# baryshnikova-lab/safepy

Hardware: AMD Instinct MI355X
Metric: node-attribute enrichments/sec (nodes x attrs x perms), compute_pvalues permutation test (higher is better)
Workload: dtype u1 (bit-sliced integer counts; f64 outputs)

## Files before the change

safepy_amd/csrc/check_hidden_regs.py:

```python
#!/usr/bin/env python3
import glob
import os
import re
import subprocess
import sys
import tempfile

LLVM = os.environ.get('SAFE_LLVM_BIN', '/opt/rocm/lib/llvm/bin')
KERNEL = '_Z19k_permtest_bits_blkILi8E'
RESERVED = range(112, 120)
OWN = re.compile(r'^(global_load_dwordx4 v\[(112:115|116:119)\], v\d+, s\[\d+:\d+\]'
                 r'|v_and_b32_e32 v\d+, 0xffff, v11[2-9]'
                 r'|v_lshrrev_b32_e32 v\d+, 16, v11[2-9])\s*$')


def names_reserved(text):
    for lo, hi in re.findall(r'\bv\[(\d+):(\d+)\]', text):
        if int(lo) <= RESERVED[-1] and int(hi) >= RESERVED[0]:
            return True
    for single in re.findall(r'\bv(\d+)\b', text):
        if int(single) in RESERVED:
            return True
    return False


def hipcc_version():
    try:
        out = subprocess.run([os.environ.get('HIPCC', '/opt/rocm/bin/hipcc'), '--version'], capture_output=True, text=True).stdout
        hip = re.search(r'HIP version: (\S+)', out)
        clang = re.search(r'clang version (\S+)', out)
        return 'hipcc %s (clang %s)' % (hip.group(1) if hip else '?', clang.group(1) if clang else '?')
    except OSError:
        return 'hipcc ?'


def write_header(path, checked, note):
    with open(path, 'w') as f:
        f.write('// generated by check_hidden_regs.py at build time\n')
        f.write('#define SAFE_HIDDEN_REGS_CHECKED %d\n' % (1 if checked else 0))
        f.write('#define SAFE_BUILD_COMPILER "%s"\n' % hipcc_version().replace('"', "'"))
        f.write('#define SAFE_BUILD_NOTE "%s"\n' % note.replace('"', "'"))


def main():
    obj, header = sys.argv[1], sys.argv[2]
    objdump, readobj = os.path.join(LLVM, 'llvm-objdump'), os.path.join(LLVM, 'llvm-readobj')
    if not os.path.exists(objdump):
        write_header(header, False, 'hidden-register check NOT run (no llvm-objdump): the kernel form without hidden registers is used')
        print('check_hidden_regs: no llvm-objdump at %s -- the library will run the form without hidden registers' % objdump)
        return 0
    with tempfile.TemporaryDirectory() as tmp:
        local = os.path.join(tmp, 'enrich.o')
        with open(obj, 'rb') as src, open(local, 'wb') as dst:
            dst.write(src.read())
        subprocess.run([objdump, '--offloading', local], capture_output=True, cwd=tmp, check=True)
        kernels, uses, foreign, vgprs = set(), 0, [], {}
        arch = os.environ.get('SAFE_ARCH', 'gfx950')
        for co in sorted(glob.glob(os.path.join(tmp, 'enrich.o.*%s*' % arch))):
            text = subprocess.run([objdump, '-d', '--no-show-raw-insn', co], capture_output=True, text=True, check=True).stdout
            if KERNEL not in text:
                continue
            sym = None
            for line in text.split('\n'):
                m = re.match(r'^[0-9a-f]+ <(.+)>:$', line)
                if m:
                    sym = m.group(1)
                    continue
                ins = line.split('//')[0].strip()
                if sym and sym.startswith(KERNEL) and names_reserved(ins):
                    kernels.add(sym)
                    uses += 1
                    if not OWN.match(ins):
                        foreign.append((sym[:60], ins))
            if os.path.exists(readobj):
                notes = subprocess.run([readobj, '--notes', co], capture_output=True, text=True).stdout
                for blk in notes.split('- .agpr_count')[1:]:
                    name = re.search(r'\.name:\s+(\S+)', blk)
                    count = re.search(r'\.vgpr_count:\s+(\d+)', blk)
                    if name and count and name.group(1).startswith(KERNEL):
                        vgprs[name.group(1)] = int(count.group(1))
    if not kernels or uses < 1000:
        print('check_hidden_regs: FAILED -- the stream kernels were not found in %s (%d uses of v112..v119)' % (obj, uses))
        return 1
    if foreign:
        print('check_hidden_regs: FAILED -- the compiler uses the reserved registers v112..v119 itself:')
        for sym, ins in foreign[:10]:
            print('   %s: %s' % (sym, ins))
        return 1
    stream = {k: v for k, v in vgprs.items() if k in kernels}
    bad = {k: v for k, v in stream.items() if v != 120}
    if bad:
        print('check_hidden_regs: FAILED -- kernel descriptors with a VGPR count other than 120: %s' % bad)
        return 1
    write_header(header, True, 'hidden-register check passed: %d kernels, %d uses of v112..v119, all the id stream\'s own; %d descriptors at 120 VGPRs'
                 % (len(kernels), uses, len(stream)))
    print('check_hidden_regs: ok (%d stream kernels, %d uses of v112..v119, %d descriptors checked)' % (len(kernels), uses, len(stream)))
    return 0


if __name__ == '__main__':
    sys.exit(main())
```

safepy_amd/csrc/enrich.hip:

```cpp
#include <algorithm>
#include <cmath>
#include <numeric>

#include "common.h"
#include "hyp_math.h"

template <typename T, int BN, int PLANES>
__global__ __launch_bounds__(256) void k_tile_prep(const void *__restrict__ raw, int64_t n, int64_t rs, int64_t cs,
                                                   int64_t col0, int64_t mloc, int64_t n_tiles,
                                                   double *__restrict__ bt) {
    const int64_t idx = static_cast<int64_t>(blockIdx.x) * 256 + threadIdx.x;
    const int64_t total = n_tiles * (n + 1) * BN;
    if (idx >= total) return;
    const int c = static_cast<int>(idx % BN);
    const int64_t row = (idx / BN) % (n + 1);
    const int64_t tile = idx / (static_cast<int64_t>(BN) * (n + 1));
    const int64_t j = tile * BN + c;
    double v = 0.0, v2 = 0.0, nn = 0.0;
    if (row < n && j < mloc) {
        const T x = reinterpret_cast<const T *>(raw)[row * rs + (col0 + j) * cs];
        if (x == x) {
            v = static_cast<double>(x);
            v2 = static_cast<double>(static_cast<T>(x * x));
            nn = 1.0;
// ... 365 lines not shown
}

#define BT_LV 10
static_assert(BT_LV == BITS_PLAN_LV, "the planning header (bits_plan.h) cuts the forms at the same number of levels");

typedef uint4 __attribute__((may_alias)) uint4_alias;

__device__ __forceinline__ uint32_t xor3(uint32_t a, uint32_t b, uint32_t c) { return __builtin_amdgcn_bitop3_b32(a, b, c, 0x96); }
__device__ __forceinline__ uint32_t maj3(uint32_t a, uint32_t b, uint32_t c) { return __builtin_amdgcn_bitop3_b32(a, b, c, 0xE8); }

template <int LV>
__device__ __forceinline__ uint32_t vadd8(uint32_t (&s)[LV], const uint32_t (&x)[8]) {
    uint32_t t2a = maj3(s[0], x[0], x[1]);
    s[0] = xor3(s[0], x[0], x[1]);
    uint32_t t2b = maj3(s[0], x[2], x[3]);
    s[0] = xor3(s[0], x[2], x[3]);
    const uint32_t t4a = maj3(s[1], t2a, t2b);
    s[1] = xor3(s[1], t2a, t2b);
    t2a = maj3(s[0], x[4], x[5]);
    s[0] = xor3(s[0], x[4], x[5]);
    t2b = maj3(s[0], x[6], x[7]);
    s[0] = xor3(s[0], x[6], x[7]);
    const uint32_t t4b = maj3(s[1], t2a, t2b);
    s[1] = xor3(s[1], t2a, t2b);
    const uint32_t t8 = maj3(s[2], t4a, t4b);
    s[2] = xor3(s[2], t4a, t4b);
    return t8;
}

template <int LV>
__device__ __forceinline__ void vripple(uint32_t (&s)[LV], uint32_t t8) {
#pragma unroll
    for (int l = 3; l < LV; ++l) {
        const uint32_t c = s[l] & t8;
        s[l] ^= t8;
        t8 = c;
    }
}

typedef const __attribute__((address_space(3))) unsigned short *lds_u16_ptr;
typedef unsigned int u32x2 __attribute__((ext_vector_type(2)));
typedef const __attribute__((address_space(3))) u32x2 *lds_u2_ptr;

template <int CL>
__device__ __forceinline__ void vcount(uint32_t (&c)[CL], uint32_t &pend, uint32_t m) {
#pragma unroll
    for (int l = 0; l < 3; ++l) {
        uint32_t k;
        asm("v_and_b32 %0, %1, %2\n\tv_xor_b32 %1, %1, %2" : "=&v"(k), "+v"(c[l]) : "v"(m));
        m = k;
    }
    pend |= m;
}

template <int CL>
__device__ __forceinline__ void vflush(uint32_t (&c)[CL], uint32_t &pend) {
    uint32_t m = pend;
#pragma unroll
    for (int l = 3; l < CL; ++l) {
        uint32_t k;
        asm("v_and_b32 %0, %1, %2\n\tv_xor_b32 %1, %1, %2" : "=&v"(k), "+v"(c[l]) : "v"(m));
        m = k;
    }
    pend = 0;
}

template <int NT = 256>
__device__ __forceinline__ void load_word_column(uint2 *__restrict__ T, const uint2 *__restrict__ src, int64_t n) {
    constexpr int UNL = NT > 256 ? 4 : 16;
    for (int64_t r0 = threadIdx.x; r0 <= n; r0 += NT * UNL) {
        uint2 v[UNL];
#pragma unroll
        for (int u = 0; u < UNL; ++u) {
            const int64_t r = r0 + u * NT;
            v[u] = src[r <= n ? r : n];
        }
#pragma unroll
        for (int u = 0; u < UNL; ++u) {
            const int64_t r = r0 + u * NT;
            if (r <= n) T[r] = v[u];
        }
    }
}

template <int LEVELS>
__device__ __forceinline__ unsigned int vextract(const uint32_t (&c)[LEVELS], int bit) {
    unsigned int v = 0;
#pragma unroll
    for (int l = 0; l < LEVELS; ++l) v |= ((c[l] >> bit) & 1u) << l;
    return v;
}

__device__ __forceinline__ void transpose32(uint32_t (&a)[32]) {
#pragma unroll
    for (int j = 16; j != 0; j >>= 1) {
        const uint32_t m = j == 16 ? 0x0000FFFFu : j == 8 ? 0x00FF00FFu : j == 4 ? 0x0F0F0F0Fu : j == 2 ? 0x33333333u : 0x55555555u;
#pragma unroll
        for (int k = 0; k < 32; ++k) {
            if ((k & j) == 0) {
                const uint32_t t = ((a[k] >> j) ^ a[k + j]) & m;
                a[k] ^= t << j;
                a[k + j] ^= t;
            }
        }
    }
}

__global__ __launch_bounds__(256) void k_permute_cols(const uint16_t *__restrict__ cur16, int64_t stride16,
                                                      const uint16_t *__restrict__ sell_col2, int64_t entries,
                                                      int64_t entries_pad, int64_t p0, int64_t count, uint32_t pad_off,
                                                      uint16_t *__restrict__ out, int sh) {
    extern __shared__ uint16_t row[];
    const int64_t q = blockIdx.y;
    if (q >= count) return;
    const uint4 *src = reinterpret_cast<const uint4 *>(cur16 + (p0 + q) * stride16);
    for (int64_t v = threadIdx.x; v < stride16 / 8; v += 256) reinterpret_cast<uint4 *>(row)[v] = src[v];
    __syncthreads();
    const int64_t e0 = static_cast<int64_t>(blockIdx.x) * 4096;
#pragma unroll
    for (int j = 0; j < 2; ++j) {
        const int64_t e = e0 + (j * 256 + threadIdx.x) * 8;
        if (e >= entries_pad) break;
        uint4 o;
        if (e + 8 <= entries) {
            const uint4 c = *reinterpret_cast<const uint4 *>(sell_col2 + e);
            const uint32_t a0 = row[(c.x & 0xFFFFu) >> 1], a1 = row[c.x >> 17], a2 = row[(c.y & 0xFFFFu) >> 1], a3 = row[c.y >> 17];
            const uint32_t a4 = row[(c.z & 0xFFFFu) >> 1], a5 = row[c.z >> 17], a6 = row[(c.w & 0xFFFFu) >> 1], a7 = row[c.w >> 17];
            o.x = (a0 << sh) | (a1 << (16 + sh));
            o.y = (a2 << sh) | (a3 << (16 + sh));
            o.z = (a4 << sh) | (a5 << (16 + sh));
            o.w = (a6 << sh) | (a7 << (16 + sh));
        } else {
            uint32_t v[8];
#pragma unroll
            for (int u = 0; u < 8; ++u) v[u] = e + u < entries ? static_cast<uint32_t>(row[sell_col2[e + u] >> 1]) << sh : pad_off;
            o.x = (v[0] & 0xFFFFu) | (v[1] << 16);
            o.y = (v[2] & 0xFFFFu) | (v[3] << 16);
            o.z = (v[4] & 0xFFFFu) | (v[5] << 16);
            o.w = (v[6] & 0xFFFFu) | (v[7] << 16);
        }
        *reinterpret_cast<uint4 *>(out + q * entries_pad + e) = o;
    }
}

template <int SHIFT, int LV>
__device__ __forceinline__ void bits_accumulate_ids(const uint16_t *__restrict__ ids, int wdt, uint32_t t_addr,
                                                    uint32_t (&s0)[LV], uint32_t (&s1)[LV]) {
#pragma unroll
    for (int l = 0; l < LV; ++l) s0[l] = s1[l] = 0;
    uint32_t c[8];
#pragma unroll
    for (int u = 0; u < 8; ++u) c[u] = ids[u * 64];
    const uint16_t *pc = ids + 8 * 64;
    for (int t0 = 0; t0 < wdt; t0 += 8, pc += 8 * 64) {
        uint32_t r[8];
#pragma unroll
        for (int u = 0; u < 8; ++u) r[u] = (c[u] << SHIFT) + t_addr;
#pragma unroll
        for (int u = 0; u < 8; ++u) c[u] = pc[u * 64];
        uint32_t x0[8], x1[8];
#pragma unroll
        for (int u = 0; u < 8; ++u) {
            const u32x2 w = *(lds_u2_ptr)(uintptr_t)(r[u]);
            x0[u] = w.x;
            x1[u] = w.y;
        }
// ... 246 lines not shown
}

template <int LV>
__device__ __forceinline__ void vripple_lv(uint32_t (&s)[LV], uint32_t t8) {
#pragma unroll
    for (int l = 3; l < LV; ++l) {
        uint32_t c;
        asm("v_and_b32 %0, %1, %2\n\tv_xor_b32 %1, %1, %2" : "=&v"(c), "+v"(s[l]) : "v"(t8));
        t8 = c;
    }
}

template <int LV>
__device__ __forceinline__ uint32_t vripple_low(uint32_t (&s)[LV], uint32_t t8) {
#pragma unroll
    for (int l = 3; l < 5 && l < LV; ++l) {
        uint32_t c;
        asm("v_and_b32 %0, %1, %2\n\tv_xor_b32 %1, %1, %2" : "=&v"(c), "+v"(s[l]) : "v"(t8));
        t8 = c;
    }
    return t8;
}
template <int LV>
__device__ __forceinline__ void vripple_high(uint32_t (&s)[LV], uint32_t t32) {
#pragma unroll
    for (int l = 5; l < LV; ++l) {
        uint32_t c;
        asm("v_and_b32 %0, %1, %2\n\tv_xor_b32 %1, %1, %2" : "=&v"(c), "+v"(s[l]) : "v"(t32));
        t32 = c;
    }
}

template <int LV, int SHIFT, int GATHER, bool RIP2 = false>
__device__ __forceinline__ void blk_add8(u32x4 &c, const u32x4 *__restrict__ refill, uint32_t (&s0)[LV], uint32_t (&s1)[LV]) {
    uint32_t a[8];
    a[0] = (c.x & 0xFFFFu) << SHIFT;
    a[1] = (c.x >> 16) << SHIFT;
    a[2] = (c.y & 0xFFFFu) << SHIFT;
    a[3] = (c.y >> 16) << SHIFT;
    a[4] = (c.z & 0xFFFFu) << SHIFT;
    a[5] = (c.z >> 16) << SHIFT;
    a[6] = (c.w & 0xFFFFu) << SHIFT;
    a[7] = (c.w >> 16) << SHIFT;
    c = *refill;
    if (GATHER == 2) {
        const uint32_t lane_bits = (__builtin_amdgcn_mbcnt_hi(~0u, __builtin_amdgcn_mbcnt_lo(~0u, 0u)) & 31u) << 3;
#pragma unroll
        for (int u = 0; u < 8; ++u) a[u] = (a[u] & 0xFF00u) | lane_bits;
    }
    uint32_t x0[8], x1[8];
#pragma unroll
    for (int u = 0; u < 8; ++u) {
        if (GATHER) {
            const u32x2 w = *(lds_u2_ptr)(uintptr_t)(a[u]);
            x0[u] = w.x;
            x1[u] = w.y;
        } else {
            x0[u] = a[u];
            x1[u] = a[u] >> 3;
        }
    }
    const uint32_t e0 = vadd8_lv<LV>(s0, x0);
    const uint32_t e1 = vadd8_lv<LV>(s1, x1);
    if (__builtin_amdgcn_ballot_w64((e0 | e1) != 0)) {
        if constexpr (RIP2 && LV >= 8) {
            const uint32_t c0 = vripple_low<LV>(s0, e0), c1 = vripple_low<LV>(s1, e1);
            if (__builtin_amdgcn_ballot_w64((c0 | c1) != 0)) {
                vripple_high<LV>(s0, c0);
                vripple_high<LV>(s1, c1);
            }
        } else {
            vripple_lv<LV>(s0, e0);
            vripple_lv<LV>(s1, e1);
        }
    }
}

#pragma clang diagnostic push
#pragma clang diagnostic ignored "-Winline-asm"
template <int Q>
__device__ __forceinline__ void stream_fetch(const u32x4 *base, uint32_t lane_off) {
    if (Q == 0) asm volatile("global_load_dwordx4 v[112:115], %0, %1" : : "v"(lane_off), "s"(base) : "v112", "v113", "v114", "v115");
    else asm volatile("global_load_dwordx4 v[116:119], %0, %1" : : "v"(lane_off), "s"(base) : "v116", "v117", "v118", "v119");
}

template <int LV, int GATHER, bool RIP2, int Q>
__device__ __forceinline__ void blk_add8s(const u32x4 *base, uint32_t lane_off, uint32_t (&s0)[LV], uint32_t (&s1)[LV]) {
    uint32_t a[8];
    if (Q == 0)
        asm volatile("s_waitcnt vmcnt(1)\n\tv_and_b32 %0, 0xffff, v112\n\tv_lshrrev_b32 %1, 16, v112\n\tv_and_b32 %2, 0xffff, v113\n\t"
                     "v_lshrrev_b32 %3, 16, v113\n\tv_and_b32 %4, 0xffff, v114\n\tv_lshrrev_b32 %5, 16, v114\n\t"
                     "v_and_b32 %6, 0xffff, v115\n\tv_lshrrev_b32 %7, 16, v115"
                     : "=v"(a[0]), "=v"(a[1]), "=v"(a[2]), "=v"(a[3]), "=v"(a[4]), "=v"(a[5]), "=v"(a[6]), "=v"(a[7]));
    else
        asm volatile("s_waitcnt vmcnt(1)\n\tv_and_b32 %0, 0xffff, v116\n\tv_lshrrev_b32 %1, 16, v116\n\tv_and_b32 %2, 0xffff, v117\n\t"
                     "v_lshrrev_b32 %3, 16, v117\n\tv_and_b32 %4, 0xffff, v118\n\tv_lshrrev_b32 %5, 16, v118\n\t"
                     "v_and_b32 %6, 0xffff, v119\n\tv_lshrrev_b32 %7, 16, v119"
                     : "=v"(a[0]), "=v"(a[1]), "=v"(a[2]), "=v"(a[3]), "=v"(a[4]), "=v"(a[5]), "=v"(a[6]), "=v"(a[7]));
    stream_fetch<Q>(base, lane_off);
    if (GATHER == 2) {
        const uint32_t lane_bits = (__builtin_amdgcn_mbcnt_hi(~0u, __builtin_amdgcn_mbcnt_lo(~0u, 0u)) & 31u) << 3;
#pragma unroll
        for (int u = 0; u < 8; ++u) a[u] = (a[u] & 0xFF00u) | lane_bits;
    }
    uint32_t x0[8], x1[8];
#pragma unroll
    for (int u = 0; u < 8; ++u) {
        if (GATHER) {
            const u32x2 w = *(lds_u2_ptr)(uintptr_t)(a[u]);
            x0[u] = w.x;
            x1[u] = w.y;
        } else {
            x0[u] = a[u];
            x1[u] = a[u] >> 3;
        }
    }
    const uint32_t e0 = vadd8_lv<LV>(s0, x0);
    const uint32_t e1 = vadd8_lv<LV>(s1, x1);
    if (__builtin_amdgcn_ballot_w64((e0 | e1) != 0)) {
        if constexpr (RIP2 && LV >= 8) {
            const uint32_t c0 = vripple_low<LV>(s0, e0), c1 = vripple_low<LV>(s1, e1);
            if (__builtin_amdgcn_ballot_w64((c0 | c1) != 0)) {
                vripple_high<LV>(s0, c0);
                vripple_high<LV>(s1, c1);
            }
        } else {
            vripple_lv<LV>(s0, e0);
            vripple_lv<LV>(s1, e1);
        }
    }
}

constexpr int HALF_MAX_LV = 8;
template <int Q>
__device__ __forceinline__ void stream_ids_lo(uint32_t (&a)[4]) {
    if (Q == 0)
        asm volatile("s_waitcnt vmcnt(1)\n\tv_and_b32 %0, 0xffff, v112\n\tv_lshrrev_b32 %1, 16, v112\n\tv_and_b32 %2, 0xffff, v113\n\t"
                     "v_lshrrev_b32 %3, 16, v113" : "=v"(a[0]), "=v"(a[1]), "=v"(a[2]), "=v"(a[3]));
    else
        asm volatile("s_waitcnt vmcnt(1)\n\tv_and_b32 %0, 0xffff, v116\n\tv_lshrrev_b32 %1, 16, v116\n\tv_and_b32 %2, 0xffff, v117\n\t"
                     "v_lshrrev_b32 %3, 16, v117" : "=v"(a[0]), "=v"(a[1]), "=v"(a[2]), "=v"(a[3]));
}
template <int Q>
__device__ __forceinline__ void stream_ids_hi(uint32_t (&a)[4]) {
    if (Q == 0)
        asm volatile("v_and_b32 %0, 0xffff, v114\n\tv_lshrrev_b32 %1, 16, v114\n\tv_and_b32 %2, 0xffff, v115\n\t"
                     "v_lshrrev_b32 %3, 16, v115" : "=v"(a[0]), "=v"(a[1]), "=v"(a[2]), "=v"(a[3]));
    else
        asm volatile("v_and_b32 %0, 0xffff, v118\n\tv_lshrrev_b32 %1, 16, v118\n\tv_and_b32 %2, 0xffff, v119\n\t"
                     "v_lshrrev_b32 %3, 16, v119" : "=v"(a[0]), "=v"(a[1]), "=v"(a[2]), "=v"(a[3]));
}
template <int GATHER>
__device__ __forceinline__ void gather4(uint32_t (&a)[4], uint32_t (&x0)[4], uint32_t (&x1)[4]) {
    if (GATHER == 2) {
        const uint32_t lane_bits = (__builtin_amdgcn_mbcnt_hi(~0u, __builtin_amdgcn_mbcnt_lo(~0u, 0u)) & 31u) << 3;
#pragma unroll
        for (int u = 0; u < 4; ++u) a[u] = (a[u] & 0xFF00u) | lane_bits;
    }
#pragma unroll
    for (int u = 0; u < 4; ++u) {
        if (GATHER) {
            const u32x2 w = *(lds_u2_ptr)(uintptr_t)(a[u]);
            x0[u] = w.x;
            x1[u] = w.y;
        } else {
            x0[u] = a[u];
            x1[u] = a[u] >> 3;
        }
    }
}
template <int LV>
__device__ __forceinline__ uint32_t vadd4_lv(uint32_t (&s)[LV], const uint32_t (&x)[4]) {
    const uint32_t t2a = maj3(s[0], x[0], x[1]);
    s[0] = xor3(s[0], x[0], x[1]);
    const uint32_t t2b = maj3(s[0], x[2], x[3]);
    s[0] = xor3(s[0], x[2], x[3]);
    const uint32_t t4 = maj3(s[1], t2a, t2b);
    s[1] = xor3(s[1], t2a, t2b);
    return t4;
}
template <int LV, int GATHER, bool RIP2, int Q>
__device__ __forceinline__ void blk_step(const u32x4 *base, uint32_t lane_off, uint32_t (&s0)[LV], uint32_t (&s1)[LV], uint32_t (&X0)[4],
                                         uint32_t (&X1)[4]) {
    uint32_t a[4], Y0[4], Y1[4];
    stream_ids_hi<Q>(a);
    stream_fetch<Q>(base, lane_off);
    gather4<GATHER>(a, Y0, Y1);
    const uint32_t f0 = vadd4_lv<LV>(s0, X0), f1 = vadd4_lv<LV>(s1, X1);
    stream_ids_lo<1 - Q>(a);
    gather4<GATHER>(a, X0, X1);
    const uint32_t h0 = vadd4_lv<LV>(s0, Y0), h1 = vadd4_lv<LV>(s1, Y1);
    const uint32_t e0 = maj3(s0[2], f0, h0), e1 = maj3(s1[2], f1, h1);
    s0[2] = xor3(s0[2], f0, h0);
    s1[2] = xor3(s1[2], f1, h1);
    if (__builtin_amdgcn_ballot_w64((e0 | e1) != 0)) {
        if constexpr (RIP2 && LV >= 8) {
            const uint32_t c0 = vripple_low<LV>(s0, e0), c1 = vripple_low<LV>(s1, e1);
            if (__builtin_amdgcn_ballot_w64((c0 | c1) != 0)) {
                vripple_high<LV>(s0, c0);
                vripple_high<LV>(s1, c1);
            }
        } else {
            vripple_lv<LV>(s0, e0);
            vripple_lv<LV>(s1, e1);
        }
    }
}

template <int LV, int SHIFT, int GATHER, bool RIP2 = false>
__device__ __forceinline__ void blk_sum(const u32x4 *__restrict__ ids, int lane, int nblk, uint32_t (&s0)[LV], uint32_t (&s1)[LV]) {
#pragma unroll
    for (int l = 0; l < LV; ++l) s0[l] = s1[l] = 0;
    u32x4 ca = ids[lane], cb = ids[64 + lane];
    const u32x4 *pc = ids + 128 + lane;
    int b = 0;
    constexpr int STEP = GATHER == 3 ? 0 : 128;
    for (; b + 1 < nblk; b += 2, pc += STEP) {
        blk_add8<LV, SHIFT, GATHER, RIP2>(ca, pc, s0, s1);
        blk_add8<LV, SHIFT, GATHER, RIP2>(cb, pc + 64, s0, s1);
    }
    if (b < nblk) blk_add8<LV, SHIFT, GATHER, RIP2>(ca, pc, s0, s1);
}

template <int LV, int CL, int DBG>
__device__ __forceinline__ void blk_task_core(const uint32_t *__restrict__ obs, const u32x4 *__restrict__ perm_ids, int64_t perm_stride,
                                              int lane, int nblk, int np, uint32_t (&g0)[CL], uint32_t (&g1)[CL], uint32_t (&l0)[CL],
                                              uint32_t (&l1)[CL]) {
    constexpr int GATHER = (DBG & 1) ? 0 : (DBG & 8) ? 2 : (DBG & 16) ? 3 : 1;
    uint32_t o0[LV], o1[LV];
#pragma unroll
    for (int l = 0; l < LV; ++l) {
        o0[l] = obs[l * 64 + lane];
        o1[l] = obs[(BT_LV + l) * 64 + lane];
    }
    uint32_t gp0 = 0, gp1 = 0, lp0 = 0, lp1 = 0;
    constexpr bool STREAM = (DBG & 256) == 0;
    u32x4 ca{}, cb{};
    const bool single = !STREAM && LV == 4 && nblk == 1 && GATHER != 3;
    if (single) {
        ca = perm_ids[lane];
        cb = perm_ids[(np > 1 ? perm_stride : 0) + lane];
    }
    const uint32_t pf_hi = static_cast<uint32_t>(__builtin_amdgcn_readfirstlane(static_cast<int>(reinterpret_cast<uint64_t>(perm_ids) >> 32)));
    const uint32_t pf_lo = static_cast<uint32_t>(__builtin_amdgcn_readfirstlane(static_cast<int>(reinterpret_cast<uint64_t>(perm_ids))));
    const u32x4 *pf_base = reinterpret_cast<const u32x4 *>((static_cast<uint64_t>(pf_hi) << 32) | static_cast<uint64_t>(pf_lo));
    uint32_t pf = 0;
    int pf_left = nblk, pf_perms = np;
    const uint32_t pf_stride = static_cast<uint32_t>(perm_stride) * 16u, pf_wrap = pf_stride - static_cast<uint32_t>(nblk) * 1024u;
    const uint32_t lane_off = static_cast<uint32_t>(lane) * 16u;
    auto pf_next = [&]() __attribute__((always_inline)) {
        if (GATHER == 3) return;
        pf += 1024u;
        if (__builtin_expect(--pf_left == 0, 0)) {
            asm volatile("");
            pf_left = nblk;
            pf += pf_wrap;
            if (--pf_perms == 0) {
                pf_perms = 1;
                pf -= pf_stride;
            }
        }
    };
    auto settle = [&](int p, uint32_t (&s0)[LV], uint32_t (&s1)[LV]) __attribute__((always_inline)) {
        if (DBG & 4) {
            g0[0] ^= s0[0] ^ s0[LV - 1];
            g1[0] ^= s1[0] ^ s1[LV - 1];
            return;
        }
        uint32_t gt0 = 0, gt1 = 0, lt0 = 0, lt1 = 0;
#pragma unroll
        for (int l = 0; l < LV; ++l) {
            lt0 = __builtin_amdgcn_bitop3_b32(s0[l], o0[l], lt0, 0x8E);
            gt0 = __builtin_amdgcn_bitop3_b32(s0[l], o0[l], gt0, 0xB2);
            lt1 = __builtin_amdgcn_bitop3_b32(s1[l], o1[l], lt1, 0x8E);
            gt1 = __builtin_amdgcn_bitop3_b32(s1[l], o1[l], gt1, 0xB2);
        }
        vcount<CL>(g0, gp0, gt0);
        vcount<CL>(g1, gp1, gt1);
        vcount<CL>(l0, lp0, lt0);
        vcount<CL>(l1, lp1, lt1);
        if ((p & 7) == 7) {
            vflush<CL>(g0, gp0);
            vflush<CL>(g1, gp1);
            vflush<CL>(l0, lp0);
            vflush<CL>(l1, lp1);
        }
    };
    if (STREAM) {
        constexpr bool R2 = (DBG & 32) == 0;
        constexpr bool HALF = (DBG & 512) == 0 && LV <= HALF_MAX_LV;
        stream_fetch<0>(pf_base, pf + lane_off);
        pf_next();
        stream_fetch<1>(pf_base, pf + lane_off);
        pf_next();
        uint32_t X0[4] = {0, 0, 0, 0}, X1[4] = {0, 0, 0, 0};
        if (HALF) {
            uint32_t a[4];
            stream_ids_lo<0>(a);
            gather4<GATHER>(a, X0, X1);
        }
        auto blockA = [&](uint32_t (&s0)[LV], uint32_t (&s1)[LV]) __attribute__((always_inline)) {
            if (HALF) blk_step<LV, GATHER, R2, 0>(pf_base, pf + lane_off, s0, s1, X0, X1);
            else blk_add8s<LV, GATHER, R2, 0>(pf_base, pf + lane_off, s0, s1);
            pf_next();
        };
        auto blockB = [&](uint32_t (&s0)[LV], uint32_t (&s1)[LV]) __attribute__((always_inline)) {
            if (HALF) blk_step<LV, GATHER, R2, 1>(pf_base, pf + lane_off, s0, s1, X0, X1);
            else blk_add8s<LV, GATHER, R2, 1>(pf_base, pf + lane_off, s0, s1);
            pf_next();
        };
        const int pairs = nblk >> 1;
        auto add_pairs = [&](uint32_t (&s0)[LV], uint32_t (&s1)[LV]) __attribute__((always_inline)) {
            for (int i = 0; i < pairs; ++i) {
                blockA(s0, s1);
                blockB(s0, s1);
            }
        };
        if (nblk & 1) {
            int p = 0;
            for (; p + 1 < np; p += 2) {
                uint32_t s0[LV], s1[LV];
#pragma unroll
                for (int l = 0; l < LV; ++l) s0[l] = s1[l] = 0;
                add_pairs(s0, s1);
                blockA(s0, s1);
                settle(p, s0, s1);
#pragma unroll
                for (int l = 0; l < LV; ++l) s0[l] = s1[l] = 0;
                blockB(s0, s1);
                add_pairs(s0, s1);
                settle(p + 1, s0, s1);
            }
            if (p < np) {
                uint32_t s0[LV], s1[LV];
#pragma unroll
                for (int l = 0; l < LV; ++l) s0[l] = s1[l] = 0;
                add_pairs(s0, s1);
                blockA(s0, s1);
                settle(p, s0, s1);
            }
        } else {
            for (int p = 0; p < np; ++p) {
                uint32_t s0[LV], s1[LV];
#pragma unroll
                for (int l = 0; l < LV; ++l) s0[l] = s1[l] = 0;
                add_pairs(s0, s1);
                settle(p, s0, s1);
            }
        }
    } else {
        for (int p = 0; p < np; ++p, perm_ids += perm_stride) {
            uint32_t s0[LV], s1[LV];
            if (single) {
#pragma unroll
                for (int l = 0; l < LV; ++l) s0[l] = s1[l] = 0;
                const u32x4 *ahead = perm_ids + (p + 2 < np ? 2 * perm_stride : 0) + lane;
                if (p & 1) blk_add8<LV, 0, GATHER>(cb, ahead, s0, s1);
                else blk_add8<LV, 0, GATHER>(ca, ahead, s0, s1);
            } else
                blk_sum<LV, 0, GATHER, (DBG & 32) == 0>(perm_ids, lane, nblk, s0, s1);
            settle(p, s0, s1);
        }
    }
    vflush<CL>(g0, gp0);
    vflush<CL>(g1, gp1);
    vflush<CL>(l0, lp0);
    vflush<CL>(l1, lp1);
    if (STREAM) asm volatile("s_waitcnt vmcnt(0)" : : : "v112", "v113", "v114", "v115", "v116", "v117", "v118", "v119");
}
#pragma clang diagnostic pop

template <int LV, int CL, int DBG>
__device__ __forceinline__ void blk_task(const uint32_t *__restrict__ obs, const u32x4 *__restrict__ perm_ids, int64_t perm_stride,
                                         int lane, int nblk, int np, uint32_t (&g0)[CL], uint32_t (&g1)[CL], uint32_t (&l0)[CL],
                                         uint32_t (&l1)[CL]) {
    blk_task_core<LV, CL, DBG>(obs, perm_ids, perm_stride, lane, nblk, np, g0, g1, l0, l1);
}

template <int LV>
__device__ __forceinline__ void observed_wave(const u32x4 *__restrict__ ids, int lane, int nblk, uint32_t *__restrict__ obs,
                                              uint32_t (&oo0)[BT_LV], uint32_t (&oo1)[BT_LV]) {
    uint32_t o0[LV], o1[LV];
    blk_sum<LV, 2, 1>(ids, lane, nblk, o0, o1);
#pragma unroll
    for (int l = 0; l < BT_LV; ++l) {
        oo0[l] = l < LV ? o0[l < LV ? l : 0] : 0u;
        oo1[l] = l < LV ? o1[l < LV ? l : 0] : 0u;
        obs[l * 64 + lane] = oo0[l];
        obs[(BT_LV + l) * 64 + lane] = oo1[l];
    }
}

__global__ __launch_bounds__(256) void k_bits_observed(int64_t n, const int32_t *__restrict__ sell_row,
                                                       const int64_t *__restrict__ slice_off,
                                                       const int32_t *__restrict__ slice_width,
                                                       const uint16_t *__restrict__ sell_col2b, int64_t n_slices,
                                                       const uint2 *__restrict__ bbits, int64_t mloc,
                                                       uint32_t *__restrict__ obs, double *__restrict__ ns_out) {
    extern __shared__ unsigned int lds[];
    uint2 *T = reinterpret_cast<uint2 *>(lds);
    if ((uint32_t)(uintptr_t)((__attribute__((address_space(3))) unsigned int *)lds) != 0u) __builtin_trap();
    const int wave = __builtin_amdgcn_readfirstlane(threadIdx.x >> 6), lane = threadIdx.x & 63;
    const int64_t wg = blockIdx.x, s = static_cast<int64_t>(blockIdx.y) * 4 + wave;
    load_word_column(T, bbits + wg * (n + 1), n);
    __syncthreads();
    if (s >= n_slices) return;
    const int wdt = __builtin_amdgcn_readfirstlane(slice_width[s]);
    const u32x4 *ids = reinterpret_cast<const u32x4 *>(sell_col2b) + slice_off[s] / 8;
    uint32_t *my_obs = obs + (wg * n_slices + s) * (2 * BT_LV * 64);
    uint32_t oo0[BT_LV], oo1[BT_LV];
    if (wdt <= 8) observed_wave<4>(ids, lane, wdt >> 3, my_obs, oo0, oo1);
    else if (wdt <= 56) observed_wave<6>(ids, lane, wdt >> 3, my_obs, oo0, oo1);
    else if (wdt <= 248) observed_wave<8>(ids, lane, wdt >> 3, my_obs, oo0, oo1);
    else if (wdt <= 504) observed_wave<9>(ids, lane, wdt >> 3, my_obs, oo0, oo1);
    else observed_wave<BT_LV>(ids, lane, wdt >> 3, my_obs, oo0, oo1);
    if (ns_out) {
        const int32_t row = sell_row[s * 64 + lane];
        uint16_t *tile = reinterpret_cast<uint16_t *>(lds + 2 * ((n + 2) & ~int64_t(1)) + 4) + wave * (64 * 66);
#pragma unroll
        for (int half = 0; half < 2; ++half)
#pragma unroll
            for (int bit = 0; bit < 32; ++bit)
                tile[lane * 66 + half * 32 + bit] = static_cast<uint16_t>(half ? vextract<BT_LV>(oo1, bit) : vextract<BT_LV>(oo0, bit));
        const int64_t jc = wg * 64 + lane;
#pragma unroll 8
        for (int r = 0; r < 64; ++r) {
            const int32_t row_r = __shfl(row, r);
            if (row_r >= 0 && jc < mloc) ns_out[static_cast<int64_t>(row_r) * mloc + jc] = static_cast<double>(tile[r * 66 + lane]);
        }
    }
}

template <int CL, bool PLAIN_STORE = false>
__device__ __forceinline__ void flush_counters(const uint32_t (&g0)[CL], const uint32_t (&g1)[CL], const uint32_t (&l0)[CL],
                                               const uint32_t (&l1)[CL], unsigned int *__restrict__ gl_counts, int64_t col0,
                                               int64_t mloc, int64_t n_pad, int64_t spos, bool active) {
#pragma unroll
    for (int half = 0; half < 2; ++half) {
        uint32_t m[32];
#pragma unroll
        for (int l = 0; l < 16; ++l) {
            m[l] = l < CL ? (half ? g1[l < CL ? l : 0] : g0[l < CL ? l : 0]) : 0u;
            m[16 + l] = l < CL ? (half ? l1[l < CL ? l : 0] : l0[l < CL ? l : 0]) : 0u;
        }
        transpose32(m);
        const int64_t c_first = col0 + half * 32;
        const int n_valid = static_cast<int>(mloc - c_first < 32 ? (mloc - c_first > 0 ? mloc - c_first : 0) : 32);
        int64_t off = c_first * n_pad + spos;
#pragma unroll
        for (int bit = 0; bit < 32; ++bit) {
            asm volatile("" : "+v"(off));
            if (PLAIN_STORE) {
                if (bit < n_valid && active && m[bit]) gl_counts[off] = m[bit];
            } else if (bit < n_valid && active && m[bit]) atomicAdd(gl_counts + off, m[bit]);
            off += n_pad;
        }
    }
}

constexpr int BLK_TRACE_MAX = 1 << 17;
__device__ unsigned long long g_blk_trace[BLK_TRACE_MAX * 8];
__device__ unsigned int g_blk_trace_n;

template <int CL, int DBG>
__device__ __forceinline__ void bits_blk_body(

    int64_t n, const uint16_t *__restrict__ ids_p, int64_t entries_pad, const int32_t *__restrict__ sell_row,
    const int64_t *__restrict__ slice_off, const int32_t *__restrict__ slice_width,
    const uint32_t *__restrict__ obs, int64_t n_slices, const uint2 *__restrict__ bbits, BitsQueues qs,
    const int4 *__restrict__ tasks, int64_t p_base, int64_t p_limit, unsigned int *__restrict__ queue, int64_t mloc,
    unsigned int *__restrict__ gl_counts, int64_t n_pad) {
    extern __shared__ unsigned int lds[];
    const int64_t t_words = 2 * ((n + 2) & ~int64_t(1));
    uint2 *T = reinterpret_cast<uint2 *>(lds);
    int *slot_box = reinterpret_cast<int *>(lds + t_words);
    if ((uint32_t)(uintptr_t)((__attribute__((address_space(3))) unsigned int *)lds) != 0u) __builtin_trap();
    const int wave = __builtin_amdgcn_readfirstlane(threadIdx.x >> 6), lane = threadIdx.x & 63;
    const int home = blockIdx.x & 7;
    int tried = 0;

    for (;;) {
        if (threadIdx.x == 0) {
            int slot = -1;
            while (tried < 8) {
                const int q = (home + tried) & 7;
                const unsigned int got = atomicAdd(queue + q, 1u);
                if (got < static_cast<unsigned int>(qs.off[q + 1] - qs.off[q])) {
                    slot = qs.off[q] + static_cast<int>(got);
                    break;
                }
                ++tried;
            }
            *slot_box = slot;
        }
        __syncthreads();
        const int slot = *slot_box;
        __syncthreads();
        if (slot < 0) break;
        const int4 task = tasks[4 * slot + wave];
        const int wg = task.x;
        const int64_t s = task.y;
        const bool active = s >= 0 && s < n_slices;
        const int64_t p_begin = p_base + task.z;
        int64_t p_end = p_base + task.w < p_limit ? p_base + task.w : p_limit;
        if (p_end < p_begin || !active) p_end = p_begin;

        unsigned long long t_begin = 0;
        if (DBG & 128) t_begin = __builtin_readcyclecounter();
        load_word_column(T, bbits + static_cast<int64_t>(wg) * (n + 1), n);
        const int64_t my_blk = (active ? slice_off[s] : 0) / 8;
        const int wdt = __builtin_amdgcn_readfirstlane(active ? slice_width[s] : 0);
        const int nblk = wdt >> 3;
        const int np = static_cast<int>(p_end - p_begin);
        const uint32_t *my_obs = obs + (static_cast<int64_t>(wg) * n_slices + (active ? s : 0)) * (2 * BT_LV * 64);
        const u32x4 *perm_ids = reinterpret_cast<const u32x4 *>(ids_p + (p_begin - p_base) * entries_pad) + my_blk;
        const int64_t perm_stride = entries_pad / 8;
        __syncthreads();
        unsigned long long t_ready = 0, t_counted = 0;
        if (DBG & 128) t_ready = __builtin_readcyclecounter();

        uint32_t g0[CL], g1[CL], l0[CL], l1[CL];
#pragma unroll
        for (int l = 0; l < CL; ++l) g0[l] = g1[l] = l0[l] = l1[l] = 0;
        if (np <= 0) {
        } else if (DBG & 1024) {
            blk_task<4, CL, DBG>(my_obs, perm_ids, perm_stride, lane, nblk, np, g0, g1, l0, l1);
        } else if (DBG & 2048) {
            blk_task<6, CL, DBG>(my_obs, perm_ids, perm_stride, lane, nblk, np, g0, g1, l0, l1);
        } else if (wdt <= 8) blk_task<4, CL, DBG>(my_obs, perm_ids, perm_stride, lane, nblk, np, g0, g1, l0, l1);
        else if (wdt <= 56) blk_task<6, CL, DBG>(my_obs, perm_ids, perm_stride, lane, nblk, np, g0, g1, l0, l1);
        else if (wdt <= 248) blk_task<8, CL, DBG>(my_obs, perm_ids, perm_stride, lane, nblk, np, g0, g1, l0, l1);
        else if (wdt <= 504) blk_task<9, CL, DBG>(my_obs, perm_ids, perm_stride, lane, nblk, np, g0, g1, l0, l1);
        else blk_task<BT_LV, CL, DBG>(my_obs, perm_ids, perm_stride, lane, nblk, np, g0, g1, l0, l1);

        if (DBG & 128) {
            asm volatile("" : "+v"(g0[0]), "+v"(l0[0]));
            t_counted = __builtin_readcyclecounter();
        }
        const int64_t spos = s * 64 + lane;
        if (!(DBG & 2)) {
            if (np > 0) flush_counters<CL, (DBG & 64) != 0>(g0, g1, l0, l1, gl_counts, static_cast<int64_t>(wg) * 64, mloc, n_pad, spos, active);
        } else if (active && (g0[0] | g1[0] | l0[0] | l1[0]) == 0xDEADBEEFu) {
            gl_counts[spos] = g0[1] ^ l0[1];
        }
        if ((DBG & 128) && lane == 0) {
            const unsigned int at = atomicAdd(&g_blk_trace_n, 1u);
            if (at < BLK_TRACE_MAX) {
                g_blk_trace[8 * at] = (static_cast<unsigned long long>(blockIdx.x) << 32) | (static_cast<unsigned long long>(slot) << 2) | wave;
                g_blk_trace[8 * at + 1] = t_begin;
                g_blk_trace[8 * at + 2] = __builtin_readcyclecounter();
                g_blk_trace[8 * at + 3] = (static_cast<unsigned long long>(nblk) << 32) | static_cast<unsigned int>(np);
                g_blk_trace[8 * at + 4] = t_ready;
                g_blk_trace[8 * at + 5] = t_counted;
            }
        }
        __syncthreads();
    }
}

template <int CL, int DBG>
__global__ __launch_bounds__(256, 4) __attribute__((amdgpu_num_vgpr(56))) void k_permtest_bits_blk(

    int64_t n, const uint16_t *__restrict__ ids_p, int64_t entries_pad, const int32_t *__restrict__ sell_row,
    const int64_t *__restrict__ slice_off, const int32_t *__restrict__ slice_width,
    const uint32_t *__restrict__ obs, int64_t n_slices, const uint2 *__restrict__ bbits, BitsQueues qs,
    const int4 *__restrict__ tasks, int64_t p_base, int64_t p_limit, unsigned int *__restrict__ queue, int64_t mloc,
    unsigned int *__restrict__ gl_counts, int64_t n_pad) {
    bits_blk_body<CL, DBG & ~256>(n, ids_p, entries_pad, sell_row, slice_off, slice_width, obs, n_slices, bbits, qs, tasks, p_base, p_limit, queue, mloc, gl_counts, n_pad);
}
template <int CL, int DBG>
__global__ __launch_bounds__(256, 4) void k_permtest_bits_blk_plain(

    int64_t n, const uint16_t *__restrict__ ids_p, int64_t entries_pad, const int32_t *__restrict__ sell_row,
    const int64_t *__restrict__ slice_off, const int32_t *__restrict__ slice_width,
    const uint32_t *__restrict__ obs, int64_t n_slices, const uint2 *__restrict__ bbits, BitsQueues qs,
    const int4 *__restrict__ tasks, int64_t p_base, int64_t p_limit, unsigned int *__restrict__ queue, int64_t mloc,
    unsigned int *__restrict__ gl_counts, int64_t n_pad) {
    bits_blk_body<CL, DBG | 256>(n, ids_p, entries_pad, sell_row, slice_off, slice_width, obs, n_slices, bbits, qs, tasks, p_base, p_limit, queue, mloc, gl_counts, n_pad);
}

constexpr int FIN_TP = 16, FIN_TC = 512;
template <bool DIRECT, int MODE, bool TAB_LDS, bool PK20 = false>
__global__ __launch_bounds__(256) void k_counts_finalize(const unsigned int *__restrict__ counts, int64_t n_pad,
                                                         const int32_t *__restrict__ sell_row,
                                                         const double *__restrict__ ns, int64_t mloc, int64_t n_perm,
                                                         PermOut out, int pv_lds) {
    __shared__ unsigned int tile[FIN_TC][FIN_TP + 1];
    __shared__ unsigned int part[4][FIN_TC];
    __shared__ int32_t rows[FIN_TP];
    extern __shared__ double tab_lds[];
    const int wave = threadIdx.x >> 6, lane = threadIdx.x & 63;
    const int64_t spos0 = static_cast<int64_t>(blockIdx.x) * FIN_TP, c0 = static_cast<int64_t>(blockIdx.y) * FIN_TC;
    {
        const int p = threadIdx.x & (FIN_TP - 1), cq = threadIdx.x / FIN_TP;
#pragma unroll
        for (int half = 0; half < 2; ++half) {
            unsigned int v[16];
#pragma unroll
            for (int k = 0; k < 16; ++k) {
                const int64_t c = c0 + cq + 16 * (half * 16 + k);
                if (PK20) {
                    const unsigned int *col = counts + (c < mloc ? c : mloc - 1) * (n_pad / 8 * 5);
                    const int64_t pos = spos0 + p, i = pos >> 1;
                    const unsigned long long x = static_cast<unsigned long long>(col[i]) |
                                                 (static_cast<unsigned long long>(reinterpret_cast<const unsigned char *>(col + n_pad / 2)[i]) << 32);
                    const unsigned int pair = static_cast<unsigned int>(x >> (20 * (pos & 1))) & 0xFFFFFu;
                    v[k] = ((pair >> 10) << 16) | (pair & 0x3FFu);
                } else {
                    v[k] = counts[(c < mloc ? c : mloc - 1) * n_pad + spos0 + p];
                }
            }
#pragma unroll
            for (int k = 0; k < 16; ++k) tile[cq + 16 * (half * 16 + k)][p] = v[k];
        }
    }
    if (threadIdx.x < FIN_TP) rows[threadIdx.x] = sell_row[spos0 + threadIdx.x];
// ... 1697 lines not shown
```

Before: 6809 billion.

## Overlap id-stream prefetch and obs loads with LDS column staging before barrier

Moves the first two hidden-register id-stream prefetches and the per-lane observed-count loads ahead of the workgroup barrier. The obs loads are issued inside the first chunk of the LDS word-column copy, and the stream position is carried in a StreamPos struct into the block task. This hides global load latency behind the LDS staging and sync, and removes compiler-placed vmcnt waits from the compare loop. The build check is extended to fail if the compiler inserts vmcnt waits in the compare blocks. The cost is higher register pressure from keeping the obs values live across the barrier, within a fixed 120-VGPR budget.

Measured after the change: 6752 billion. Within noise of the previous version (-0.8%).

```diff
diff --git a/safepy_amd/csrc/check_hidden_regs.py b/safepy_amd/csrc/check_hidden_regs.py
--- a/safepy_amd/csrc/check_hidden_regs.py
+++ b/safepy_amd/csrc/check_hidden_regs.py
@@ -22,6 +22,51 @@
         if int(single) in RESERVED:
             return True
     return False
+
+
+LABEL = re.compile(r'^[0-9a-f]+ <(.+)>:$')
+BLOCK_END = re.compile(r'^(s_cbranch_\w+|s_branch|s_endpgm|s_setpc_b64)\b')
+COMPARE = re.compile(r'^v_bitop3_b32 .*bitop3:0x(8e|b2)\b')
+VM_WAIT = re.compile(r'^s_waitcnt\b.*\bvmcnt\(\d+\)')
+STREAM_WAIT = re.compile(r'^s_waitcnt vmcnt\(1\)\s*$')
+EXTRACT = re.compile(r'^(v_and_b32_e32 v\d+, 0xffff|v_lshrrev_b32_e32 v\d+, 16), v11[2-9]\s*$')
+
+
+def stream_wait_violations(text, kernel=KERNEL):
+    blocks, cur, sym = [], [], None
+
+    def close():
+        if cur and sym and sym.startswith(kernel):
+            blocks.append((sym, list(cur)))
+        del cur[:]
+
+    for line in text.split('\n'):
+        m = LABEL.match(line.strip())
+        if m:
+            close()
+            if not re.match(r'^L\d+$', m.group(1)):
+                sym = m.group(1)
+            continue
+        ins = line.split('//')[0].strip()
+        if not ins:
+            continue
+        cur.append(ins)
+        if BLOCK_END.match(ins):
+            close()
+    close()
+    compare_blocks, own, bad = 0, 0, []
+    for name, body in blocks:
+        if not any(COMPARE.match(i) for i in body):
+            continue
+        compare_blocks += 1
+        for k, ins in enumerate(body):
+            if not VM_WAIT.match(ins):
+                continue
+            if STREAM_WAIT.match(ins) and k + 1 < len(body) and EXTRACT.match(body[k + 1]):
+                own += 1
+            else:
+                bad.append((name, body[max(0, k - 2):k + 2]))
+    return compare_blocks, own, bad
 
 
 def hipcc_version():
@@ -55,6 +100,7 @@
             dst.write(src.read())
         subprocess.run([objdump, '--offloading', local], capture_output=True, cwd=tmp, check=True)
         kernels, uses, foreign, vgprs = set(), 0, [], {}
+        cmp_blocks, own_waits, wait_bad = 0, 0, []
         arch = os.environ.get('SAFE_ARCH', 'gfx950')
         for co in sorted(glob.glob(os.path.join(tmp, 'enrich.o.*%s*' % arch))):
             text = subprocess.run([objdump, '-d', '--no-show-raw-insn', co], capture_output=True, text=True, check=True).stdout
@@ -72,6 +118,10 @@
                     uses += 1
                     if not OWN.match(ins):
                         foreign.append((sym[:60], ins))
+            labelled = subprocess.run([objdump, '-d', '--no-show-raw-insn', '--symbolize-operands', co], capture_output=True, text=True,
+                                      check=True).stdout
+            found = stream_wait_violations(labelled)
+            cmp_blocks, own_waits, wait_bad = cmp_blocks + found[0], own_waits + found[1], wait_bad + found[2]
             if os.path.exists(readobj):
                 notes = subprocess.run([readobj, '--notes', co], capture_output=True, text=True).stdout
                 for blk in notes.split('- .agpr_count')[1:]:
@@ -92,9 +142,22 @@
     if bad:
         print('check_hidden_regs: FAILED -- kernel descriptors with a VGPR count other than 120: %s' % bad)
         return 1
-    write_header(header, True, 'hidden-register check passed: %d kernels, %d uses of v112..v119, all the id stream\'s own; %d descriptors at 120 VGPRs'
-                 % (len(kernels), uses, len(stream)))
-    print('check_hidden_regs: ok (%d stream kernels, %d uses of v112..v119, %d descriptors checked)' % (len(kernels), uses, len(stream)))
+    if cmp_blocks == 0:
+        print('check_hidden_regs: FAILED -- no basic block with the compare truth tables found in the stream kernels')
+        return 1
+    if wait_bad:
+        print('check_hidden_regs: FAILED -- %d compiler-placed vmcnt waits in the compare blocks of the stream kernels (they drain the id '
+              'stream\'s prefetches in every permutation):' % len(wait_bad))
+        for sym, lines in wait_bad[:10]:
+            print('   %s:' % sym[:60])
+            for ins in lines:
+                print('      %s' % ins)
+        return 1
+    write_header(header, True, 'hidden-register check passed: %d kernels, %d uses of v112..v119, all the id stream\'s own; %d descriptors at 120 VGPRs; '
+                 'stream-wait check passed: %d compare blocks, no vmcnt wait but the stream\'s own %d'
+                 % (len(kernels), uses, len(stream), cmp_blocks, own_waits))
+    print('check_hidden_regs: ok (%d stream kernels, %d uses of v112..v119, %d descriptors checked; %d compare blocks, 0 compiler vmcnt '
+          'waits in them, %d of the stream\'s own)' % (len(kernels), uses, len(stream), cmp_blocks, own_waits))
     return 0
 
 
diff --git a/safepy_amd/csrc/enrich.hip b/safepy_amd/csrc/enrich.hip
--- a/safepy_amd/csrc/enrich.hip
+++ b/safepy_amd/csrc/enrich.hip
@@ -471,6 +471,28 @@
         }
     }
 }
+template <class F>
+__device__ __forceinline__ void load_word_column_then(uint2 *__restrict__ T, const uint2 *__restrict__ src, int64_t n, uint32_t tid, F &&between) {
+    constexpr int UNL = 16, NT = 256;
+    auto chunk = [&](int64_t r0, auto &&mid) __attribute__((always_inline)) {
+        uint2 v[UNL];
+#pragma unroll
+        for (int u = 0; u < UNL; ++u) {
+            const int64_t r = r0 + u * NT;
+            v[u] = src[r <= n ? r : n];
+        }
+        __builtin_amdgcn_sched_barrier(0);
+        mid();
+        __builtin_amdgcn_sched_barrier(0);
+#pragma unroll
+        for (int u = 0; u < UNL; ++u) {
+            const int64_t r = r0 + u * NT;
+            T[r <= n ? r : n] = v[u];
+        }
+    };
+    chunk(tid, between);
+    for (int64_t r0 = static_cast<int64_t>(tid) + NT * UNL; r0 <= n; r0 += NT * UNL) chunk(r0, [] {});
+}
 
 template <int LEVELS>
 __device__ __forceinline__ unsigned int vextract(const uint32_t (&c)[LEVELS], int bit) {
@@ -883,6 +905,48 @@
 __device__ __forceinline__ void stream_fetch(const u32x4 *base, uint32_t lane_off) {
     if (Q == 0) asm volatile("global_load_dwordx4 v[112:115], %0, %1" : : "v"(lane_off), "s"(base) : "v112", "v113", "v114", "v115");
     else asm volatile("global_load_dwordx4 v[116:119], %0, %1" : : "v"(lane_off), "s"(base) : "v116", "v117", "v118", "v119");
+}
+
+struct StreamPos {
+    const u32x4 *base;
+    uint32_t pf;
+    int left, perms;
+    uint32_t stride, wrap;
+    int nblk;
+};
+template <int GATHER>
+__device__ __forceinline__ void stream_next(StreamPos &sp) {
+    if (GATHER == 3) return;
+    sp.pf += 1024u;
+    if (__builtin_expect(--sp.left == 0, 0)) {
+        asm volatile("");
+        sp.left = sp.nblk;
+        sp.pf += sp.wrap;
+        if (--sp.perms == 0) {
+            sp.perms = 1;
+            sp.pf -= sp.stride;
+        }
+    }
+}
+template <int GATHER>
+__device__ __forceinline__ StreamPos stream_begin(const u32x4 *perm_ids, int64_t perm_stride, int lane, int nblk, int np) {
+    StreamPos sp;
+    const uint32_t pf_hi = static_cast<uint32_t>(__builtin_amdgcn_readfirstlane(static_cast<int>(reinterpret_cast<uint64_t>(perm_ids) >> 32)));
+    const uint32_t pf_lo = static_cast<uint32_t>(__builtin_amdgcn_readfirstlane(static_cast<int>(reinterpret_cast<uint64_t>(perm_ids))));
+    sp.base = reinterpret_cast<const u32x4 *>((static_cast<uint64_t>(pf_hi) << 32) | static_cast<uint64_t>(pf_lo));
+    sp.pf = 0;
+    sp.left = nblk;
+    sp.perms = np;
+    sp.stride = static_cast<uint32_t>(perm_stride) * 16u;
+    sp.wrap = sp.stride - static_cast<uint32_t>(nblk) * 1024u;
+    sp.nblk = nblk;
+    const uint32_t lane_off = static_cast<uint32_t>(lane) * 16u;
+    asm volatile("s_nop 4");
+    stream_fetch<0>(sp.base, sp.pf + lane_off);
+    stream_next<GATHER>(sp);
+    stream_fetch<1>(sp.base, sp.pf + lane_off);
+    stream_next<GATHER>(sp);
+    return sp;
 }
 
 template <int LV, int GATHER, bool RIP2, int Q>
@@ -1024,15 +1088,17 @@
 }
 
 template <int LV, int CL, int DBG>
-__device__ __forceinline__ void blk_task_core(const uint32_t *__restrict__ obs, const u32x4 *__restrict__ perm_ids, int64_t perm_stride,
+__device__ __forceinline__ void blk_task_core(const uint32_t (&ob0)[BT_LV], const uint32_t (&ob1)[BT_LV], StreamPos sp,
+                                              const u32x4 *__restrict__ perm_ids, int64_t perm_stride,
                                               int lane, int nblk, int np, uint32_t (&g0)[CL], uint32_t (&g1)[CL], uint32_t (&l0)[CL],
                                               uint32_t (&l1)[CL]) {
     constexpr int GATHER = (DBG & 1) ? 0 : (DBG & 8) ? 2 : (DBG & 16) ? 3 : 1;
     uint32_t o0[LV], o1[LV];
 #pragma unroll
     for (int l = 0; l < LV; ++l) {
-        o0[l] = obs[l * 64 + lane];
-        o1[l] = obs[(BT_LV + l) * 64 + lane];
+        o0[l] = ob0[l];
+        o1[l] = ob1[l];
+        asm volatile("" : : "v"(o0[l]), "v"(o1[l]));
     }
     uint32_t gp0 = 0, gp1 = 0, lp0 = 0, lp1 = 0;
     constexpr bool STREAM = (DBG & 256) == 0;
@@ -1042,26 +1108,9 @@
         ca = perm_ids[lane];
         cb = perm_ids[(np > 1 ? perm_stride : 0) + lane];
     }
-    const uint32_t pf_hi = static_cast<uint32_t>(__builtin_amdgcn_readfirstlane(static_cast<int>(reinterpret_cast<uint64_t>(perm_ids) >> 32)));
-    const uint32_t pf_lo = static_cast<uint32_t>(__builtin_amdgcn_readfirstlane(static_cast<int>(reinterpret_cast<uint64_t>(perm_ids))));
-    const u32x4 *pf_base = reinterpret_cast<const u32x4 *>((static_cast<uint64_t>(pf_hi) << 32) | static_cast<uint64_t>(pf_lo));
-    uint32_t pf = 0;
-    int pf_left = nblk, pf_perms = np;
-    const uint32_t pf_stride = static_cast<uint32_t>(perm_stride) * 16u, pf_wrap = pf_stride - static_cast<uint32_t>(nblk) * 1024u;
+    const u32x4 *pf_base = sp.base;
     const uint32_t lane_off = static_cast<uint32_t>(lane) * 16u;
-    auto pf_next = [&]() __attribute__((always_inline)) {
-        if (GATHER == 3) return;
-        pf += 1024u;
-        if (__builtin_expect(--pf_left == 0, 0)) {
-            asm volatile("");
-            pf_left = nblk;
-            pf += pf_wrap;
-            if (--pf_perms == 0) {
-                pf_perms = 1;
-                pf -= pf_stride;
-            }
-        }
-    };
+    auto pf_next = [&]() __attribute__((always_inline)) { stream_next<GATHER>(sp); };
     auto settle = [&](int p, uint32_t (&s0)[LV], uint32_t (&s1)[LV]) __attribute__((always_inline)) {
         if (DBG & 4) {
             g0[0] ^= s0[0] ^ s0[LV - 1];
@@ -1090,10 +1139,6 @@
     if (STREAM) {
         constexpr bool R2 = (DBG & 32) == 0;
         constexpr bool HALF = (DBG & 512) == 0 && LV <= HALF_MAX_LV;
-        stream_fetch<0>(pf_base, pf + lane_off);
-        pf_next();
-        stream_fetch<1>(pf_base, pf + lane_off);
-        pf_next();
         uint32_t X0[4] = {0, 0, 0, 0}, X1[4] = {0, 0, 0, 0};
         if (HALF) {
             uint32_t a[4];
@@ -1101,13 +1146,13 @@
             gather4<GATHER>(a, X0, X1);
         }
         auto blockA = [&](uint32_t (&s0)[LV], uint32_t (&s1)[LV]) __attribute__((always_inline)) {
-            if (HALF) blk_step<LV, GATHER, R2, 0>(pf_base, pf + lane_off, s0, s1, X0, X1);
-            else blk_add8s<LV, GATHER, R2, 0>(pf_base, pf + lane_off, s0, s1);
+            if (HALF) blk_step<LV, GATHER, R2, 0>(pf_base, sp.pf + lane_off, s0, s1, X0, X1);
+            else blk_add8s<LV, GATHER, R2, 0>(pf_base, sp.pf + lane_off, s0, s1);
             pf_next();
         };
         auto blockB = [&](uint32_t (&s0)[LV], uint32_t (&s1)[LV]) __attribute__((always_inline)) {
-            if (HALF) blk_step<LV, GATHER, R2, 1>(pf_base, pf + lane_off, s0, s1, X0, X1);
-            else blk_add8s<LV, GATHER, R2, 1>(pf_base, pf + lane_off, s0, s1);
+            if (HALF) blk_step<LV, GATHER, R2, 1>(pf_base, sp.pf + lane_off, s0, s1, X0, X1);
+            else blk_add8s<LV, GATHER, R2, 1>(pf_base, sp.pf + lane_off, s0, s1);
             pf_next();
         };
         const int pairs = nblk >> 1;
@@ -1172,10 +1217,11 @@
 #pragma clang diagnostic pop
 
 template <int LV, int CL, int DBG>
-__device__ __forceinline__ void blk_task(const uint32_t *__restrict__ obs, const u32x4 *__restrict__ perm_ids, int64_t perm_stride,
+__device__ __forceinline__ void blk_task(const uint32_t (&ob0)[BT_LV], const uint32_t (&ob1)[BT_LV], const StreamPos &sp,
+                                         const u32x4 *__restrict__ perm_ids, int64_t perm_stride,
                                          int lane, int nblk, int np, uint32_t (&g0)[CL], uint32_t (&g1)[CL], uint32_t (&l0)[CL],
                                          uint32_t (&l1)[CL]) {
-    blk_task_core<LV, CL, DBG>(obs, perm_ids, perm_stride, lane, nblk, np, g0, g1, l0, l1);
+    blk_task_core<LV, CL, DBG>(ob0, ob1, sp, perm_ids, perm_stride, lane, nblk, np, g0, g1, l0, l1);
 }
 
 template <int LV>
@@ -1276,7 +1322,7 @@
     uint2 *T = reinterpret_cast<uint2 *>(lds);
     int *slot_box = reinterpret_cast<int *>(lds + t_words);
     if ((uint32_t)(uintptr_t)((__attribute__((address_space(3))) unsigned int *)lds) != 0u) __builtin_trap();
-    const int wave = __builtin_amdgcn_readfirstlane(threadIdx.x >> 6), lane = threadIdx.x & 63;
+    const int wave = __builtin_amdgcn_readfirstlane(threadIdx.x >> 6);
     const int home = blockIdx.x & 7;
     int tried = 0;
 
@@ -1308,31 +1354,46 @@
 
         unsigned long long t_begin = 0;
         if (DBG & 128) t_begin = __builtin_readcyclecounter();
-        load_word_column(T, bbits + static_cast<int64_t>(wg) * (n + 1), n);
+        uint32_t tid = threadIdx.x;
+        asm volatile("" : "+v"(tid));
+        const int lane = static_cast<int>(tid & 63u);
+        const uint32_t *my_obs = obs + (static_cast<int64_t>(wg) * n_slices + (active ? s : 0)) * (2 * BT_LV * 64);
+        uint32_t ob0[BT_LV], ob1[BT_LV];
+        load_word_column_then(T, bbits + static_cast<int64_t>(wg) * (n + 1), n, tid, [&]() __attribute__((always_inline)) {
+#pragma unroll
+            for (int l = 0; l < BT_LV; ++l) {
+                ob0[l] = my_obs[l * 64 + lane];
+                ob1[l] = my_obs[(BT_LV + l) * 64 + lane];
+            }
+        });
         const int64_t my_blk = (active ? slice_off[s] : 0) / 8;
         const int wdt = __builtin_amdgcn_readfirstlane(active ? slice_width[s] : 0);
         const int nblk = wdt >> 3;
         const int np = static_cast<int>(p_end - p_begin);
-        const uint32_t *my_obs = obs + (static_cast<int64_t>(wg) * n_slices + (active ? s : 0)) * (2 * BT_LV * 64);
         const u32x4 *perm_ids = reinterpret_cast<const u32x4 *>(ids_p + (p_begin - p_base) * entries_pad) + my_blk;
         const int64_t perm_stride = entries_pad / 8;
+        constexpr int GATHER = (DBG & 1) ? 0 : (DBG & 8) ? 2 : (DBG & 16) ? 3 : 1;
+        StreamPos sp{};
+        if ((DBG & 256) == 0 && np > 0) sp = stream_begin<GATHER>(perm_ids, perm_stride, lane, nblk, np);
         __syncthreads();
         unsigned long long t_ready = 0, t_counted = 0;
         if (DBG & 128) t_ready = __builtin_readcyclecounter();
+#pragma unroll
+        for (int l = 0; l < BT_LV; ++l) asm volatile("" : : "v"(ob0[l]), "v"(ob1[l]));
 
         uint32_t g0[CL], g1[CL], l0[CL], l1[CL];
 #pragma unroll
         for (int l = 0; l < CL; ++l) g0[l] = g1[l] = l0[l] = l1[l] = 0;
         if (np <= 0) {
         } else if (DBG & 1024) {
-            blk_task<4, CL, DBG>(my_obs, perm_ids, perm_stride, lane, nblk, np, g0, g1, l0, l1);
+            blk_task<4, CL, DBG>(ob0, ob1, sp, perm_ids, perm_stride, lane, nblk, np, g0, g1, l0, l1);
         } else if (DBG & 2048) {
-            blk_task<6, CL, DBG>(my_obs, perm_ids, perm_stride, lane, nblk, np, g0, g1, l0, l1);
-        } else if (wdt <= 8) blk_task<4, CL, DBG>(my_obs, perm_ids, perm_stride, lane, nblk, np, g0, g1, l0, l1);
-        else if (wdt <= 56) blk_task<6, CL, DBG>(my_obs, perm_ids, perm_stride, lane, nblk, np, g0, g1, l0, l1);
-        else if (wdt <= 248) blk_task<8, CL, DBG>(my_obs, perm_ids, perm_stride, lane, nblk, np, g0, g1, l0, l1);
-        else if (wdt <= 504) blk_task<9, CL, DBG>(my_obs, perm_ids, perm_stride, lane, nblk, np, g0, g1, l0, l1);
-        else blk_task<BT_LV, CL, DBG>(my_obs, perm_ids, perm_stride, lane, nblk, np, g0, g1, l0, l1);
+            blk_task<6, CL, DBG>(ob0, ob1, sp, perm_ids, perm_stride, lane, nblk, np, g0, g1, l0, l1);
+        } else if (wdt <= 8) blk_task<4, CL, DBG>(ob0, ob1, sp, perm_ids, perm_stride, lane, nblk, np, g0, g1, l0, l1);
+        else if (wdt <= 56) blk_task<6, CL, DBG>(ob0, ob1, sp, perm_ids, perm_stride, lane, nblk, np, g0, g1, l0, l1);
+        else if (wdt <= 248) blk_task<8, CL, DBG>(ob0, ob1, sp, perm_ids, perm_stride, lane, nblk, np, g0, g1, l0, l1);
+        else if (wdt <= 504) blk_task<9, CL, DBG>(ob0, ob1, sp, perm_ids, perm_stride, lane, nblk, np, g0, g1, l0, l1);
+        else blk_task<BT_LV, CL, DBG>(ob0, ob1, sp, perm_ids, perm_stride, lane, nblk, np, g0, g1, l0, l1);
 
         if (DBG & 128) {
             asm volatile("" : "+v"(g0[0]), "+v"(l0[0]));
```
